# JiLiBIT/LIO-SLAM

Measured on AMD Instinct MI355X. Metric: scan-to-map registrations/sec, 64x1800 scan vs 200-keyframe map; pose RMSE, higher is better.
Workload: dtype f32

## Files before the change

### include/liogpu.h

```cpp
#ifndef LIOGPU_H
#define LIOGPU_H

#include <stddef.h>
#include <stdint.h>

#ifdef __cplusplus
extern "C" {
#endif

#define LIO_VERSION 102
#define LIO_MAX_ITERS 32

enum {
    LIO_OK               = 0,
    LIO_TOO_FEW_POINTS   = 1,
    LIO_TOO_FEW_CORR     = 2,
    LIO_ERR_ARG          = -1,
    LIO_ERR_HIP          = -2,
    LIO_ERR_CAPACITY     = -3,
    LIO_ERR_NO_MAP       = -4,
    LIO_ERR_NO_DEVICE    = -5
};

typedef struct lio_s2m_config {
// ... 99 lines not shown
void  lio_host_free(void *p);
int   lio_host_register(void *p, size_t bytes);
int   lio_host_unregister(void *p);
void *lio_device_alloc(int32_t device_id, size_t bytes);
void  lio_device_free(int32_t device_id, void *p);
int   lio_device_upload(int32_t device_id, void *dst, const void *src, size_t bytes);

int  lio_s2m_set_degeneracy(lio_s2m_handle *h, int32_t scan, const float matP[36], int32_t is_degenerate);

int  lio_s2m_get_correspondences(lio_s2m_handle *h, int32_t scan, uint8_t *flag,
                                 float *coeff4, int32_t *nn_idx5);

int  lio_s2m_set_corner_map(lio_s2m_handle *h, const void *pts, size_t n, size_t stride_bytes);
int  lio_s2m_batch_upload_corners(lio_s2m_handle *h, int32_t n_scans, const void *const *scans,
                                  const size_t *n_pts, size_t stride_bytes);
int  lio_s2m_register_cs(lio_s2m_handle *h, const void *corner_scan, size_t n_corner,
                         const void *surf_scan, size_t n_surf, size_t stride_bytes,
                         float pose[6], lio_s2m_result *res);
int  lio_s2m_get_corner_correspondences(lio_s2m_handle *h, int32_t scan, uint8_t *flag,
                                        float *coeff4, int32_t *nn_idx5);

int  lio_s2m_get_profile(lio_s2m_handle *h, lio_s2m_profile *out);
int  lio_s2m_debug_persist_spin(lio_s2m_handle *h, int32_t spin_max, int32_t withhold_wg);
int  lio_s2m_debug_stamps(lio_s2m_handle *h, long long *out, size_t cap_entries);

int  lio_s2m_set_stream(lio_s2m_handle *h, void *hip_stream);
int  lio_s2m_set_global_grid(lio_s2m_handle *h, const float origin[3], const int32_t dims[3]);
int  lio_s2m_set_shard(lio_s2m_handle *h, int32_t axis, int32_t lo, int32_t hi);
int  lio_s2m_set_shard_plan(lio_s2m_handle *h, int32_t axis, int32_t n_ranks, int32_t rank, const int32_t *bounds,
                            int32_t halo_cells);
int  lio_s2m_set_scan_shard(lio_s2m_handle *h, int32_t rank, int32_t world);
int  lio_s2m_batch_begin(lio_s2m_handle *h);
int  lio_s2m_batch_iter_partial(lio_s2m_handle *h, double *d_sums );
int  lio_s2m_batch_iter_apply(lio_s2m_handle *h, const double *d_sums);
int  lio_s2m_batch_n_active(lio_s2m_handle *h, int32_t *n_active);
int  lio_s2m_batch_poll_active(lio_s2m_handle *h, int32_t iteration, int32_t *n_active);

void lio_transform_update(float pose[6], int32_t imu_available, int32_t imu_type,
                          float imu_roll_init, float imu_pitch_init, float imu_rpy_weight,
                          float rotation_tollerance, float z_tollerance);

typedef struct lio_deskew_config {
    int32_t N_SCAN;
    int32_t downsampleRate;
    int32_t point_filter_num;
    float   lidarMinFront, lidarMinBack, lidarMinLeft, lidarMinRight;
// ... 113 lines not shown
```

### lio-slam_amd/api.py

```python
import ctypes as C
import os
import subprocess

import numpy as np

_HERE = os.path.dirname(os.path.abspath(__file__))
LIO_MAX_ITERS = 32
STATUS_NAMES = {0: "OK", 1: "TOO_FEW_POINTS", 2: "TOO_FEW_CORR", -1: "ERR_ARG", -2: "ERR_HIP",
                -3: "ERR_CAPACITY", -4: "ERR_NO_MAP", -5: "ERR_NO_DEVICE"}


class LioError(RuntimeError):
    pass


class S2MConfig(C.Structure):
    _fields_ = [
        ("k", C.c_int32), ("max_sq_dist", C.c_float),
        ("plane_tol", C.c_double), ("weight", C.c_double), ("min_s", C.c_double),
        ("min_corr", C.c_int32), ("max_iters", C.c_int32), ("eig_thresh", C.c_float),
        ("conv_deg", C.c_double), ("conv_cm", C.c_double),
        ("min_scan_pts", C.c_int32), ("jacobian_mode", C.c_int32), ("force_all_iters", C.c_int32),
        ("device_id", C.c_int32), ("cell_size", C.c_float), ("max_batch", C.c_int32),
        ("max_scan_pts", C.c_int32), ("record_corr_iter", C.c_int32), ("kernel_variant", C.c_int32),
# ... 72 lines not shown
    if verbose:
        print(out.stdout)
    return lib_path()


_LIB = None

EXPORTS = [
    "lio_version", "lio_s2m_default_config", "lio_last_error", "lio_s2m_create", "lio_s2m_destroy",
    "lio_s2m_set_map", "lio_s2m_register", "lio_s2m_batch_upload", "lio_s2m_batch_set_poses",
    "lio_s2m_batch_run", "lio_s2m_batch_sync", "lio_s2m_batch_results", "lio_s2m_set_degeneracy",
    "lio_s2m_get_correspondences", "lio_s2m_get_profile", "lio_s2m_set_stream",
    "lio_s2m_set_global_grid", "lio_s2m_set_shard", "lio_s2m_batch_begin",
    "lio_s2m_batch_iter_partial", "lio_s2m_batch_iter_apply", "lio_s2m_batch_n_active",
    "lio_transform_update", "lio_deskew_default_config", "lio_imu_deskew_info", "lio_deskew",
    "lio_curvature", "lio_s2m_debug_stamps", "lio_s2m_batch_poll_active", "lio_voxel_grid", "lio_assemble_map", "lio_kf_store_create", "lio_kf_store_destroy", "lio_kf_store_add",
    "lio_kf_store_count", "lio_kf_store_points", "lio_assemble_map_resident", "lio_s2m_set_scan_shard",
    "lio_s2m_set_corner_map", "lio_s2m_batch_upload_corners", "lio_s2m_register_cs",
    "lio_s2m_get_corner_correspondences", "lio_feature_default_config", "lio_extract_features",
    "lio_range_image_default_config", "lio_range_image",
    "lio_s2m_share_map", "lio_s2m_batch_upload_async", "lio_host_alloc", "lio_host_free", "lio_host_register",
    "lio_host_unregister", "lio_s2m_set_shard_plan", "lio_s2m_register_pc2", "lio_deskew_pc2", "lio_kf_store_add_device", "lio_kf_store_add_from_handle",
    "lio_s2m_register_raw", "lio_s2m_debug_persist_spin", "lio_device_alloc", "lio_device_free", "lio_device_upload",
    "lio_nearby_default_config", "lio_kf_store_set_poses", "lio_assemble_map_nearby",
]


def load_library():
    global _LIB
    if _LIB is not None:
        return _LIB
    p = lib_path()
    if not os.path.exists(p):
        raise LioError(f"{p} is missing: run __graft_entry__.build() (hipcc --offload-arch=gfx950). "
                       "There is no CPU fallback.")
    L = C.CDLL(p)
    vp, i32, f32, f64, sz = C.c_void_p, C.c_int32, C.c_float, C.c_double, C.c_size_t
    L.lio_version.restype = C.c_int
    L.lio_last_error.restype = C.c_char_p
    L.lio_s2m_default_config.argtypes = [C.POINTER(S2MConfig)]
    L.lio_s2m_default_config.restype = None
    L.lio_s2m_create.argtypes = [C.POINTER(S2MConfig), C.POINTER(vp)]
    L.lio_s2m_destroy.argtypes = [vp]
    L.lio_s2m_destroy.restype = None
    L.lio_s2m_set_map.argtypes = [vp, vp, sz, sz]
    L.lio_s2m_register.argtypes = [vp, vp, sz, sz, C.POINTER(f32), C.POINTER(S2MResult)]
    L.lio_s2m_register_pc2.argtypes = [vp, vp, sz, C.POINTER(PC2Layout), C.POINTER(f32), C.POINTER(S2MResult)]
# ... 421 lines not shown
                            dp(T), dp(RX), dp(RY), dp(RZ), cur, out.ctypes.data, 32, C.byref(n_out)), "lio_deskew_pc2")
    o = out[:n_out.value]
    return np.concatenate([o[:, :3], o[:, 4:5]], axis=1).copy()


def deskew_default_config(**kw):
    c = DeskewConfig()
    load_library().lio_deskew_default_config(C.byref(c))
    for k, v in kw.items():
        setattr(c, k, v)
    return c


def curvature(rng, device_id=0):
    r = np.ascontiguousarray(rng, np.float32)
    curv = np.zeros(len(r), np.float32)
    picked = np.full(len(r), -1, np.int32)
    label = np.full(len(r), -1, np.int32)
    _check(load_library().lio_curvature(device_id, r.ctypes.data, len(r), curv.ctypes.data,
                                        picked.ctypes.data, label.ctypes.data), "lio_curvature")
    return curv, picked, label


def range_image(records, t_cur, imu, device_id=0, **cfg_overrides):
    L = load_library()
    cfg = RangeImageConfig()
    L.lio_range_image_default_config(C.byref(cfg))
    cfg.device_id = device_id
    for k, v in cfg_overrides.items():
        if not hasattr(cfg, k):
            raise AttributeError(k)
        setattr(cfg, k, v)
    cur, T, RX, RY, RZ = imu
    rec = np.ascontiguousarray(records)
    cells = int(cfg.N_SCAN) * int(cfg.Horizon_SCAN)
    out = _scratch("ri_cloud", (max(cells, 1), 8))
    col = _scratch("ri_col", (max(cells, 1),), np.int32)
    rng = _scratch("ri_range", (max(cells, 1),))
    start = np.zeros(cfg.N_SCAN, np.int32)
    end = np.zeros(cfg.N_SCAN, np.int32)
    n_out = C.c_size_t()
    dpp = lambda a: a.ctypes.data_as(C.POINTER(C.c_double))
    _check(L.lio_range_image(C.byref(cfg), rec.ctypes.data, len(rec), rec.dtype.itemsize, t_cur, dpp(T), dpp(RX), dpp(RY), dpp(RZ),
                             cur, out.ctypes.data, 32, C.byref(n_out), start.ctypes.data, end.ctypes.data, col.ctypes.data,
                             rng.ctypes.data), "lio_range_image")
    n = n_out.value
# ... 156 lines not shown
```

### lio-slam_amd/csrc/lio_device_math.h

```cpp
#pragma once
#include <hip/hip_runtime.h>
#include <float.h>
#include <stdint.h>

#define LIO_DEV __device__ __forceinline__

LIO_DEV void lio_plane_qr5x3(float a[5][3], float x[3])
{
    float hc[3], direct[3], upd[3];
    int trans[3];
#pragma unroll
    for (int k = 0; k < 3; ++k) {
        float s = 0.0f;
#pragma unroll
        for (int i = 0; i < 5; ++i) s += a[i][k] * a[i][k];
        direct[k] = sqrtf(s);
        upd[k] = direct[k];
    }
    float maxn = upd[0];
    if (upd[1] > maxn) maxn = upd[1];
    if (upd[2] > maxn) maxn = upd[2];
    const float th = maxn * FLT_EPSILON;
    const float threshold_helper = (th * th) / 5.0f;
    const float downdate_thr = sqrtf(FLT_EPSILON);
    int nz = 3;

#pragma unroll
    for (int k = 0; k < 3; ++k) {
// ... 10 lines not shown
            const bool sw = (big == j);
#pragma unroll
            for (int i = 0; i < 5; ++i) {
                const float u = a[i][k], v = a[i][j];
                a[i][k] = sw ? v : u;
                a[i][j] = sw ? u : v;
            }
            const float u0 = upd[k], u1 = upd[j], d0 = direct[k], d1 = direct[j];
            upd[k] = sw ? u1 : u0;       upd[j] = sw ? u0 : u1;
            direct[k] = sw ? d1 : d0;    direct[j] = sw ? d0 : d1;
        }
        float tail_sq = 0.0f;
#pragma unroll
        for (int i = k + 1; i < 5; ++i) tail_sq += a[i][k] * a[i][k];
        const float c0 = a[k][k];
        float beta, tau;
        if (tail_sq <= FLT_MIN) {
            tau = 0.0f; beta = c0;
#pragma unroll
            for (int i = k + 1; i < 5; ++i) a[i][k] = 0.0f;
        } else {
            beta = sqrtf(c0 * c0 + tail_sq);
            if (c0 >= 0.0f) beta = -beta;
            const float den = c0 - beta;
#pragma unroll
            for (int i = k + 1; i < 5; ++i) a[i][k] = a[i][k] / den;
            tau = (beta - c0) / beta;
        }
        hc[k] = tau;
        a[k][k] = beta;
        if (tau != 0.0f) {
#pragma unroll
            for (int j = k + 1; j < 3; ++j) {
                float tmp = 0.0f;
#pragma unroll
                for (int i = k + 1; i < 5; ++i) tmp += a[i][k] * a[i][j];
                tmp += a[k][j];
                a[k][j] -= tau * tmp;
#pragma unroll
                for (int i = k + 1; i < 5; ++i) a[i][j] -= (tau * a[i][k]) * tmp;
            }
        }
#pragma unroll
        for (int j = k + 1; j < 3; ++j) {
            if (upd[j] != 0.0f) {
                float temp = fabsf(a[k][j]) / upd[j];
                temp = (1.0f + temp) * (1.0f - temp);
                temp = temp < 0.0f ? 0.0f : temp;
                const float ratio = upd[j] / direct[j];
// ... 37 lines not shown
                tmp += c[k];
                c[k] -= tau * tmp;
#pragma unroll
                for (int i = k + 1; i < 5; ++i) c[i] -= (tau * a[i][k]) * tmp;
            }
        }
    }
#pragma unroll
    for (int i = 2; i >= 0; --i) {
        if (i < nz) {
            if (c[i] != 0.0f) {
                c[i] /= a[i][i];
#pragma unroll
                for (int r = 0; r < i; ++r) c[r] -= c[i] * a[r][i];
            }
        }
    }
    const float v0 = (0 < nz) ? c[0] : 0.0f;
    const float v1 = (1 < nz) ? c[1] : 0.0f;
    const float v2 = (2 < nz) ? c[2] : 0.0f;
#pragma unroll
    for (int j = 0; j < 3; ++j)
        x[j] = (p0 == j) ? v0 : (p1 == j) ? v1 : (p2 == j) ? v2 : 0.0f;
}

LIO_DEV void lio_jacobian_row(const float tr[6], float px, float py, float pz,
                              float cx, float cy, float cz, float cw, int jac_exact,
                              float row[6], float &rhs)
{
    const float srx = tr[0], crx = tr[1], sry = tr[2], cry = tr[3], srz = tr[4], crz = tr[5];
    const float arx = (-srx * cry * px - (srx * sry * srz + crx * crz) * py + (crx * srz - srx * sry * crz) * pz) * cx
                    + (crx * cry * px - (srx * crz - crx * sry * srz) * py + (crx * sry * crz + srx * srz) * pz) * cy;
    const float mid = jac_exact ? (srx * cry * srz * py) : (srx * sry * srz * py);
    const float ary = (-crx * sry * px + crx * cry * srz * py + crx * cry * crz * pz) * cx
                    + (-srx * sry * px + mid + srx * cry * crz * pz) * cy
                    + (-cry * px - sry * srz * py - sry * crz * pz) * cz;
    const float arz = ((crx * sry * crz + srx * srz) * py + (srx * crz - crx * sry * srz) * pz) * cx
                    + ((-crx * srz + srx * sry * crz) * py + (-srx * sry * srz - crx * crz) * pz) * cy
                    + (cry * crz * py - cry * srz * pz) * cz;
    row[0] = arz; row[1] = ary; row[2] = arx;
    row[3] = cx;  row[4] = cy;  row[5] = cz;
    rhs = -cw;
}

__device__ static float lio_cv_hypot(float a, float b)
{
// ... 369 lines not shown
```

### lio-slam_amd/csrc/lio_kernels.h

```cpp
#pragma once
#include <hip/hip_runtime.h>
#include "lio_types.h"

struct LioIterParams {
    LioGrid grid;
    LioShard shard;
    LioConsts c;
    const float4* map_sorted;
    const float4* map_xyz4;
    const int* cell_start;
    const float4* nbr_pts;
    const int* nbr_start;
    const float* sx;
    const float* sy;
    const float* sz;
    const int* perm;
    LioScanState* state;
    const LioBlockDesc* blocks;
    double* partials;
    unsigned* arrive;
    int max_blk;
    int xcd_remap;
    int* n_active;
    double* sums_out;
// ... 17 lines not shown
                           int* n_active, hipStream_t s);
void lio_launch_iterate(const LioIterParams& P, int n_blocks, int ppt, bool stage, hipStream_t s, bool corner = false);
void lio_launch_persist(const LioIterParams& P, int n_blocks, unsigned* gen, unsigned epoch, const unsigned char* stage, size_t stride,
                        int n_scans, unsigned* spec, double* spec_sums, const float* poses0, unsigned spin_max, int withhold_wg, hipStream_t s);
void lio_launch_pack_summary(const LioScanState* st, int n_scans, float* out, hipStream_t s);
void lio_launch_apply(LioScanState* st, int n_scans, const double* sums, size_t slot_stride, int n_slots, const LioConsts& c,
                      int* n_active, hipStream_t s);
void lio_launch_shard_cull(const LioIterParams& P, int n_ranks, int rank, int halo, const int* bounds, const float* block_box,
                           int n_blocks, unsigned char* skip, hipStream_t s);
void lio_launch_block_boxes(const LioBlockDesc* blocks, int n_blocks, const LioScanState* st, const float* sx, const float* sy,
                            const float* sz, float* box, hipStream_t s);
void lio_launch_scan_sort_lds(const void* stage, size_t stride, const LioScanState* st, int n_scans, int max_pts, float tile0,
                              int shard_axis, int* perm, float* x, float* y, float* z, hipStream_t s);
void lio_launch_scan_bbox(const void* stage, size_t stride, const LioBlockDesc* prep_blocks, int n_prep_blocks,
                          const LioScanState* st, unsigned* bbox, hipStream_t s);
void lio_launch_scan_tile_sort(const void* stage, size_t stride, int total_pts,
                               const LioBlockDesc* prep_blocks, int n_prep_blocks,
                               const LioScanState* st, const LioScanTiles* tiles, int n_keys,
                               int* key_of, int* key_count, int* key_start, int* tile_sums,
                               int* tmp_idx, int* perm, int* big_list, int* big_cnt,
                               float* x, float* y, float* z, hipStream_t s);
void lio_launch_exclusive_scan(const int* in, int n, int* tile_sums, int* out, hipStream_t s);
void lio_launch_xyzi4_to_soa(const float4* src, int n, float* x, float* y, float* z, float4* xyz4, hipStream_t s);
```

### lio-slam_amd/csrc/lio_kernels.hip

```cpp
#include <hip/hip_runtime.h>
#include "lio_types.h"
#include "lio_device_math.h"
#include "lio_kernels.h"

#include "lio_s2m_device.h"
#include "lio_scan2.h"

LIO_DEV unsigned lio_f2ord(float f)
{
    unsigned u = __float_as_uint(f);
    return (u & 0x80000000u) ? ~u : (u | 0x80000000u);
}

__global__ void k_aos_to_soa(const unsigned char* __restrict__ src, size_t stride, int n,
                             float* __restrict__ x, float* __restrict__ y, float* __restrict__ z,
                             float4* __restrict__ xyz4 )
{
    int i = blockIdx.x * blockDim.x + threadIdx.x;
    if (i >= n) return;
    const float* p = reinterpret_cast<const float*>(src + (size_t)i * stride);
    const float a = p[0], b = p[1], c = p[2];
    x[i] = a; y[i] = b; z[i] = c;
    if (xyz4) xyz4[i] = make_float4(a, b, c, 0.0f);
}
// ... 704 lines not shown
__global__ __launch_bounds__(LIO_BLOCK, (PPT == 1 && !STAGE && !CORNER) ? LIO_MIN_WAVES : 4) void k_s2m_iterate(LioIterParams P)
{
    __shared__ __attribute__((aligned(16))) double s_rows[LIO_BLOCK][8];
    __shared__ double s_part[8][28];
    __shared__ double s_sum[28];
    __shared__ LioSolveWs s_ws;
    __shared__ __attribute__((aligned(16))) float4 s_pts[STAGE ? LIO_LDS_PTS : 1];
    __shared__ int s_cell[STAGE ? LIO_LDS_CELLS : 1];
    __shared__ int s_row_beg[STAGE ? LIO_LDS_ROWS : 1];
    __shared__ int s_row_off[STAGE ? LIO_LDS_ROWS + 1 : 1];
    __shared__ int s_box[8];
    __shared__ int s_scan4[4];

    int wg = blockIdx.x;
    if (P.xcd_remap) {
        const int n8 = gridDim.x >> 3;
        if (wg < n8 * 8) wg = (wg & 7) * n8 + (wg >> 3);
    }
    const int wg_mode = P.blk_skip != nullptr ? (int)P.blk_skip[wg] : 0;
    if (wg_mode == 1) return;
    const LioBlockDesc bd = P.blocks[wg];
    LioScanState* st = &P.state[bd.scan];
    if (st->done) return;
    long long* stamp = P.stamps ? P.stamps + ((size_t)wg * (LIO_BLOCK / 64) + (threadIdx.x >> 6)) * 8 : nullptr;
#define LIO_STAMP(k) do { if (stamp && (threadIdx.x & 63) == 0) stamp[k] = (long long)__builtin_readcyclecounter(); } while (0)
    LIO_STAMP(0);

    float T[12], tr[6];
#pragma unroll
    for (int k = 0; k < 12; ++k) T[k] = st->T[k];
#pragma unroll
    for (int k = 0; k < 6; ++k) tr[k] = st->trig[k];
    const int n_pts = CORNER ? st->c_n_pts : st->n_pts;
    const int base = CORNER ? st->c_offset : st->offset;
    const bool record = (P.rec_flag != nullptr) && (st->iter == P.c.record_iter);
    const bool use_cache = (P.d5_cache != nullptr) && !STAGE && st->iter > 0;
    float Tp[12];
#pragma unroll
    for (int k = 0; k < 12; ++k) Tp[k] = use_cache ? st->Tp[k] : 0.0f;
    const LioGrid g = P.grid;
    const int lane = threadIdx.x & 63, wave = threadIdx.x >> 6;

    float px[PPT], py[PPT], pz[PPT], qx[PPT], qy[PPT], qz[PPT];
    int cx[PPT], cy[PPT], cz[PPT];
    bool act[PPT], inr[PPT];
    int bmn[3] = { 0x7fffffff, 0x7fffffff, 0x7fffffff }, bmx[3] = { -0x7fffffff, -0x7fffffff, -0x7fffffff };
#pragma unroll
    for (int pp = 0; pp < PPT; ++pp) {
        const int li = bd.first + pp * LIO_BLOCK + (int)threadIdx.x;
        inr[pp] = li < n_pts;
        const int gi = base + (inr[pp] ? li : 0);
        px[pp] = P.sx[gi]; py[pp] = P.sy[gi]; pz[pp] = P.sz[gi];
        qx[pp] = T[0] * px[pp] + T[1] * py[pp] + T[2]  * pz[pp] + T[3];
        qy[pp] = T[4] * px[pp] + T[5] * py[pp] + T[6]  * pz[pp] + T[7];
        qz[pp] = T[8] * px[pp] + T[9] * py[pp] + T[10] * pz[pp] + T[11];
        bool a = inr[pp];
        if (P.shard.axis >= 0 && wg_mode != 2) {
            const float qa = P.shard.axis == 0 ? qx[pp] : (P.shard.axis == 1 ? qy[pp] : qz[pp]);
            int gc = lio_cell_coord(qa, P.shard.gorigin, P.shard.inv_cell, P.shard.gdim);
            gc = min(max(gc, 0), P.shard.gdim - 1);
            a = a && gc >= P.shard.lo && gc < P.shard.hi;
        }
// ... 80 lines not shown
                }
                for (int i = threadIdx.x; i < total; i += LIO_BLOCK) {
                    int lo = 0, hi = n_rows - 1;
                    while (lo < hi) {
                        const int mid = (lo + hi + 1) >> 1;
                        if (s_row_off[mid] <= i) lo = mid; else hi = mid - 1;
                    }
                    s_pts[i] = P.map_sorted[s_row_beg[lo] + (i - s_row_off[lo])];
                }
                staged = true;
            }
            __syncthreads();
        }
    }

    const int red_g = threadIdx.x >> 5, red_s = threadIdx.x & 31;
    const int red_a = c_pair_a[red_s], red_b = c_pair_b[red_s];
    double red_acc = 0.0;
    LIO_STAMP(1);

#pragma unroll 1
    for (int pp = 0; pp < PPT; ++pp) {
        float bound2 = P.c.max_sq_dist;
        float Rx = sqrtf(P.c.max_sq_dist) * 1.0001f + 1e-6f;
        bool bounded = false;
        const int ci = base + bd.first + pp * LIO_BLOCK + (int)threadIdx.x;
        if (use_cache && act[pp]) {
            const float d5 = P.d5_cache[ci];
            if (d5 >= 0.0f) {
                const float ox = Tp[0] * px[pp] + Tp[1] * py[pp] + Tp[2]  * pz[pp] + Tp[3];
                const float oy = Tp[4] * px[pp] + Tp[5] * py[pp] + Tp[6]  * pz[pp] + Tp[7];
                const float oz = Tp[8] * px[pp] + Tp[9] * py[pp] + Tp[10] * pz[pp] + Tp[11];
                const float mv = sqrtf(lio_sqdist(qx[pp], qy[pp], qz[pp], ox, oy, oz));
                const float R = (sqrtf(d5) + mv) * 1.0001f + 1e-6f;
                const float r2 = R * R * 1.0001f;
                if (r2 < bound2) { bound2 = r2; Rx = R; bounded = true; }
            }
        }
        const double sentinel = lio_make_key(bound2, -1);
        LioTop5 top = { sentinel, sentinel, sentinel, sentinel, sentinel };
        if (act[pp]) {
            if (STAGE && staged)
                lio_knn_lds(s_pts, s_cell, rxn1, ryn, rx0, ry0, rz0, ry1, rz1, g.nx, g.k,
                            qx[pp], qy[pp], qz[pp], cx[pp], cy[pp], cz[pp], top);
            else
                lio_knn_global(P, g, qx[pp], qy[pp], qz[pp], cy[pp], cz[pp], Rx, bound2, bounded, top);
        }
// ... 29 lines not shown
        __syncthreads();
        if (red_s < 28) {
#pragma unroll 8
            for (int p = red_g; p < LIO_BLOCK; p += 8)
                red_acc = __builtin_fma(s_rows[p][red_a], s_rows[p][red_b], red_acc);
        }
    }
    LIO_STAMP(4);
    if (red_s < 28) s_part[red_g][red_s] = red_acc;
    __syncthreads();
    LIO_STAMP(5);
    if (wave != 0) return;

    double* part = P.partials + ((size_t)bd.scan * P.max_blk + bd.blk) * LIO_SUMS;
    if (lane < 28) {
        double v = s_part[0][lane];
#pragma unroll
        for (int w = 1; w < 8; ++w) v += s_part[w][lane];
        __hip_atomic_store(part + lane, v, __ATOMIC_RELAXED, __HIP_MEMORY_SCOPE_AGENT);
    }
    lio_arrive_and_finish(P, bd, st, lane, s_sum, &s_ws, stamp);
    LIO_STAMP(7);
#undef LIO_STAMP
}

__global__ void k_s2m_pack_summary(const LioScanState* __restrict__ st, int n_scans, float* __restrict__ out)
{
    const int s = blockIdx.x * blockDim.x + threadIdx.x;
    if (s >= n_scans) return;
    float* o = out + (size_t)s * 10;
    for (int k = 0; k < 6; ++k) o[k] = st[s].pose[k];
    o[6] = __int_as_float(st[s].iter); o[7] = __int_as_float(st[s].status | (st[s].done ? 0 : 0x100));
    o[8] = __int_as_float(st[s].converged); o[9] = __int_as_float(st[s].is_degenerate);
}

__global__ void k_s2m_apply(LioScanState* __restrict__ st, int n_scans, const double* __restrict__ sums, size_t slot_stride, int n_slots,
                            LioConsts c, int* __restrict__ n_active)
{
    const int s = blockIdx.x;
    if (s >= n_scans) return;
    if (st[s].done) return;
    __shared__ LioSolveWs s_ws;
    __shared__ double s_tot[LIO_SUMS];
    const int lane = (int)threadIdx.x;
    if (lane < LIO_SUMS) {
        const double* p = sums + (size_t)s * LIO_SUMS + lane;
// ... 205 lines not shown
```

### lio-slam_amd/csrc/lio_persist.hip

```cpp
#include <hip/hip_runtime.h>
#ifndef LIO_PREFETCH
#define LIO_PREFETCH 2
#endif
#include "lio_kernels.h"
#include "lio_device_math.h"
#include "lio_s2m_device.h"

namespace {

__global__ __launch_bounds__(LIO_BLOCK, 2) void k_s2m_persist(LioIterParams P, unsigned* __restrict__ gen, unsigned epoch, const unsigned char* __restrict__ stage, unsigned stride,
                   int n_main, unsigned* __restrict__ spec, double* __restrict__ spec_sums, const float* __restrict__ poses0,
                   unsigned spin_max, int withhold_wg)
{
    __shared__ __attribute__((aligned(16))) double s_rows[LIO_BLOCK][8];
    __shared__ double s_part[8][28];
    __shared__ double s_sum[28];
    __shared__ LioSolveWs s_ws;
    __shared__ int s_ctl;

    const int wg = blockIdx.x;
    if (wg >= n_main) {
        const int scan = wg - n_main;
        if (threadIdx.x >= 64) return;
        const int hl = threadIdx.x;
// ... 72 lines not shown
        float T[12], tr[6], Tp[12];
#pragma unroll
        for (int k = 0; k < 12; ++k) T[k] = st->T[k];
#pragma unroll
        for (int k = 0; k < 6; ++k) tr[k] = st->trig[k];
        const int st_iter = st->iter;
        const bool record = (P.rec_flag != nullptr) && (st_iter == P.c.record_iter);
        const bool use_cache = (P.d5_cache != nullptr) && st_iter > 0;
#pragma unroll
        for (int k = 0; k < 12; ++k) Tp[k] = use_cache ? st->Tp[k] : 0.0f;

        const float qx = T[0] * px + T[1] * py + T[2]  * pz + T[3];
        const float qy = T[4] * px + T[5] * py + T[6]  * pz + T[7];
        const float qz = T[8] * px + T[9] * py + T[10] * pz + T[11];
        const int cx = lio_cell_coord(qx, g.ox, g.inv_cell, g.nx);
        const int cy = lio_cell_coord(qy, g.oy, g.inv_cell, g.ny);
        const int cz = lio_cell_coord(qz, g.oz, g.inv_cell, g.nz);
        bool act = inr;
        act = act && (fabsf(qx) <= 3.0e38f) && (fabsf(qy) <= 3.0e38f) && (fabsf(qz) <= 3.0e38f);
        act = act && cx >= -g.k && cx < g.nx + g.k && cy >= -g.k && cy < g.ny + g.k && cz >= -g.k && cz < g.nz + g.k;

        LIO_TICK(0);
        float bound2 = P.c.max_sq_dist;
        float Rx = sqrtf(P.c.max_sq_dist) * 1.0001f + 1e-6f;
        bool bounded = false;
        if (use_cache && act) {
            const float d5 = P.d5_cache[ci];
            if (d5 >= 0.0f) {
                const float ox = Tp[0] * px + Tp[1] * py + Tp[2]  * pz + Tp[3];
                const float oy = Tp[4] * px + Tp[5] * py + Tp[6]  * pz + Tp[7];
                const float oz = Tp[8] * px + Tp[9] * py + Tp[10] * pz + Tp[11];
                const float mv = sqrtf(lio_sqdist(qx, qy, qz, ox, oy, oz));
                const float R = (sqrtf(d5) + mv) * 1.0001f + 1e-6f;
                const float r2 = R * R * 1.0001f;
                if (r2 < bound2) { bound2 = r2; Rx = R; bounded = true; }
            }
        }
        const double sentinel = lio_make_key(bound2, -1);
        LioTop5 top = { sentinel, sentinel, sentinel, sentinel, sentinel };
        if (act) lio_knn_global(P, g, qx, qy, qz, cy, cz, Rx, bound2, bounded, top);
        const bool ok = act && (lio_key_d2(top.k4) < P.c.max_sq_dist);
        const int nn[5] = { lio_key_idx(top.k0), lio_key_idx(top.k1), lio_key_idx(top.k2), lio_key_idx(top.k3), lio_key_idx(top.k4) };
        if (P.d5_cache && inr) P.d5_cache[ci] = ok ? lio_key_d2(top.k4) : -1.0f;
        LIO_TICK(1);

        float cxx = 0.0f, cyy = 0.0f, czz = 0.0f, cww = 0.0f;
        bool accept = false;
// ... 150 lines not shown
```

### lio-slam_amd/csrc/lio_s2m_device.h

```cpp
#pragma once
#include <hip/hip_runtime.h>
#include "lio_types.h"
#include "lio_device_math.h"
#include "lio_kernels.h"

#define LIO_MAX_COORD 1.0e15f
#ifndef LIO_PREFETCH
#define LIO_PREFETCH 1
#endif
#ifndef LIO_ARRIVE_ACQREL
#define LIO_ARRIVE_ACQREL 0
#endif
#define LIO_IDX_MASK 0x1fffffff

LIO_DEV int lio_cell_coord(float v, float origin, float inv_cell, int n)
{
    float c = floorf((v - origin) * inv_cell);
    c = fminf(fmaxf(c, -4.0f), (float)(n + 3));
    return (int)c;
}

LIO_DEV double lio_dmin(double a, double b) { double r; asm("v_min_f64 %0, %1, %2" : "=v"(r) : "v"(a), "v"(b)); return r; }
LIO_DEV double lio_dmax(double a, double b) { double r; asm("v_max_f64 %0, %1, %2" : "=v"(r) : "v"(a), "v"(b)); return r; }

// ... 154 lines not shown
    return 0;
}

typedef float lio_f2 __attribute__((ext_vector_type(2)));

LIO_DEV void lio_knn_pair(const float4& a, const float4& b, lio_f2 qx, lio_f2 qy, lio_f2 qz, double& k0, double& k1)
{
    const lio_f2 X = { a.x, a.y }, Y = { a.z, a.w }, Z = { b.x, b.y };
    const lio_f2 dx = X - qx, dy = Y - qy, dz = Z - qz;
    const lio_f2 d2 = (dx * dx + dy * dy) + dz * dz;
    k0 = lio_make_key(d2.x, __float_as_int(b.z));
    k1 = lio_make_key(d2.y, __float_as_int(b.w));
}

LIO_DEV void lio_knn_group(const float4& c0, const float4& c1, const float4& c2, const float4& c3,
                           lio_f2 qx, lio_f2 qy, lio_f2 qz, LioTop5& top)
{
    double k0, k1, k2, k3;
    lio_knn_pair(c0, c1, qx, qy, qz, k0, k1);
    lio_knn_pair(c2, c3, qx, qy, qz, k2, k3);
    lio_top5_insert4(top, k0, k1, k2, k3);
}

LIO_DEV void lio_knn_range(const LioIterParams& P, const LioGrid& g, float qx, float qy, float qz,
                           int cy, int cz, float Rx, unsigned& beg, unsigned& end)
{
    const int xlo = lio_cell_coord(qx - Rx, g.ox, g.inv_cell_x, g.nxf), xhi = lio_cell_coord(qx + Rx, g.ox, g.inv_cell_x, g.nxf);
    const int x0 = max(xlo, 0), x1 = min(xhi, g.nxf - 1);
    beg = end = 0;
    if (x0 > x1) return;
    int row = (min(max(cz, 0), g.nz - 1) * g.ny + min(max(cy, 0), g.ny - 1)) * g.nxf;
#pragma unroll
    for (int l = 0; l < LIO_TB_MAX; ++l) {
        if (Rx <= g.tb_reach[l]) {
            const int by = min(max(lio_cell_coord(qy, g.tb_oy[l], g.tb_inv_cell[l], g.tb_ny[l]), 0), g.tb_ny[l] - 1);
            const int bz = min(max(lio_cell_coord(qz, g.tb_oz[l], g.tb_inv_cell[l], g.tb_nz[l]), 0), g.tb_nz[l] - 1);
            row = g.tb_row0[l] + (bz * g.tb_ny[l] + by) * g.nxf;
        }
    }
#if LIO_PREFETCH == 3
    beg = (unsigned)P.nbr_start[row + x0] & ~7u;
#else
    beg = (unsigned)P.nbr_start[row + x0] & ~3u;
#endif
    end = (unsigned)P.nbr_start[row + x1 + 1];
}

LIO_DEV void lio_knn_run(const LioIterParams& P, unsigned beg, unsigned end, float qx, float qy, float qz, LioTop5& top)
{
    if (beg >= end) return;
    const lio_f2 QX = { qx, qx }, QY = { qy, qy }, QZ = { qz, qz };
    const float4* p = P.nbr_pts + beg;
#if LIO_PREFETCH == 2
    float4 c0 = p[0], c1 = p[1], c2 = p[2], c3 = p[3];
    float4 n0 = p[4], n1 = p[5], n2 = p[6], n3 = p[7];
    for (unsigned j = beg;;) {
        float4 f0 = n0, f1 = n1, f2 = n2, f3 = n3;
        if (j + 8 < end) { f0 = p[8]; f1 = p[9]; f2 = p[10]; f3 = p[11]; }
        lio_knn_group(c0, c1, c2, c3, QX, QY, QZ, top);
        j += 4;
        if (j >= end) break;
        p += 4;
// ... 12 lines not shown
        const float4 b0 = p[4], b1 = p[5], b2 = p[6], b3 = p[7];
        lio_knn_group(a0, a1, a2, a3, QX, QY, QZ, top);
        p += 8;
        a0 = p[0]; a1 = p[1]; a2 = p[2]; a3 = p[3];
        lio_knn_group(b0, b1, b2, b3, QX, QY, QZ, top);
        j += 8;
    } while (j < end);
#else
    float4 c0 = p[0], c1 = p[1], c2 = p[2], c3 = p[3];
    for (unsigned j = beg + 4; j < end; j += 4) {
        p += 4;
        const float4 n0 = p[0], n1 = p[1], n2 = p[2], n3 = p[3];
        lio_knn_group(c0, c1, c2, c3, QX, QY, QZ, top);
        c0 = n0; c1 = n1; c2 = n2; c3 = n3;
    }
    lio_knn_group(c0, c1, c2, c3, QX, QY, QZ, top);
#endif
}

LIO_DEV void lio_knn_global(const LioIterParams& P, const LioGrid& g, float qx, float qy, float qz,
                            int cy, int cz, float Rx, float bound2, bool bounded, LioTop5& top)
{
    int lvl = bounded ? -1 : g.tb_try;
    for (;;) {
        float rx = Rx, b2 = bound2;
        if (lvl >= 0) {
            rx = lvl == 2 ? g.tb_reach[2] : (lvl == 1 ? g.tb_reach[1] : g.tb_reach[0]);
            b2 = lvl == 2 ? g.tb_try_b2[2] : (lvl == 1 ? g.tb_try_b2[1] : g.tb_try_b2[0]);
        }
        const double sentinel = lio_make_key(b2, -1);
        top.k0 = top.k1 = top.k2 = top.k3 = top.k4 = sentinel;
        unsigned beg, end;
        lio_knn_range(P, g, qx, qy, qz, cy, cz, rx, beg, end);
        lio_knn_run(P, beg, end, qx, qy, qz, top);
        if (lvl < 0 || lio_key_idx(top.k4) != -1) break;
        --lvl;
    }
}

template <bool CORNER>
LIO_DEV bool lio_assoc_point(const LioIterParams& P, const int nn[5], float qx, float qy, float qz,
                             float px, float py, float pz, float& cxx, float& cyy, float& czz, float& cww)
{
    bool accept = false;
    float a[5][3], m[5][3];
#pragma unroll
    for (int j = 0; j < 5; ++j) {
        const float4 mp = P.map_xyz4[nn[j]];
        m[j][0] = a[j][0] = mp.x;
        m[j][1] = a[j][1] = mp.y;
        m[j][2] = a[j][2] = mp.z;
    }
    if (CORNER) {
        accept = lio_corner_assoc(m, qx, qy, qz, P.c.weight, P.c.min_s, cxx, cyy, czz, cww);
    } else {
        float X0[3];
        lio_plane_qr5x3(a, X0);
        float pa = X0[0], pb = X0[1], pc = X0[2], pd = 1;
        const float ps = sqrtf(pa * pa + pb * pb + pc * pc);
        pa /= ps; pb /= ps; pc /= ps; pd /= ps;
        bool planeValid = true;
#pragma unroll
        for (int j = 0; j < 5; ++j) {
            const float v = fabsf(pa * m[j][0] + pb * m[j][1] + pc * m[j][2] + pd);
            if ((double)v > P.c.plane_tol) planeValid = false;
        }
        if (planeValid) {
            const float pd2 = pa * qx + pb * qy + pc * qz + pd;
            const float r2 = px * px + py * py + pz * pz;
            const float s = (float)(1 - P.c.weight * (double)fabsf(pd2) / (double)sqrtf(sqrtf(r2)));
            cxx = s * pa; cyy = s * pb; czz = s * pc; cww = s * pd2;
            accept = (double)s > P.c.min_s;
        }
    }
    return accept;
}

static __constant__ int c_pair_a[32] = { 0,0,0,0,0,0, 1,1,1,1,1, 2,2,2,2, 3,3,3, 4,4, 5,  0,1,2,3,4,5, 7, 0,0,0,0 };
static __constant__ int c_pair_b[32] = { 0,1,2,3,4,5, 1,2,3,4,5, 2,3,4,5, 3,4,5, 4,5, 5,  6,6,6,6,6,6, 7, 0,0,0,0 };

LIO_DEV void lio_arrive_and_finish(const LioIterParams& P, const LioBlockDesc& bd, LioScanState* st, int lane,
                                   double* s_sum, LioSolveWs* s_ws, long long* stamp)
{
#if !LIO_ARRIVE_ACQREL
    asm volatile("s_waitcnt vmcnt(0)" ::: "memory");
#endif
    int last = 0;
    if (lane == 0) {
#if LIO_ARRIVE_ACQREL
// ... 31 lines not shown
```

### lio-slam_amd/csrc/lio_types.h

```cpp
#pragma once
#include <stdint.h>

#define LIO_SUMS 32
#define LIO_SUM_NC 27
#define LIO_BLOCK 256
#define LIO_ROW_ALIGN 8

#define LIO_TB_MAX 3
struct LioGrid {
    float ox, oy, oz;
    float inv_cell;
    int32_t nx, ny, nz;
    int32_t n_cells;
    int32_t k;
    int32_t xs;
    int32_t nxf;
    float inv_cell_x;
    int32_t tb_row0[LIO_TB_MAX], tb_ny[LIO_TB_MAX], tb_nz[LIO_TB_MAX];
    float tb_oy[LIO_TB_MAX], tb_oz[LIO_TB_MAX], tb_inv_cell[LIO_TB_MAX], tb_reach[LIO_TB_MAX];
    int32_t tb_try;
    float tb_try_b2[LIO_TB_MAX];
};

struct LioShard {
    float gorigin;
    float inv_cell;
    int32_t axis;
    int32_t gdim;
    int32_t lo, hi;
};

struct LioConsts {
    double plane_tol, weight, min_s, conv_deg, conv_cm;
    float  max_sq_dist, eig_thresh;
    int32_t min_corr, max_iters, jac_exact, force_all, record_iter, min_scan_pts;
};

struct LioScanState {
    float pose[6];
    float T[12];
    float Tp[12];
    float trig[6];
    int32_t n_pts;
    int32_t offset;
    int32_t c_n_pts;
    int32_t c_offset;
    int32_t iter;
    int32_t done;
    int32_t converged;
    int32_t is_degenerate;
    int32_t n_corr_last;
    int32_t status;
    float matP[36];
    float AtA[36];
    float AtB[6];
    int32_t n_corr_iter[32];
    float pose_iter[32][6];
// ... 17 lines not shown
```

### lio-slam_amd/csrc/liogpu_api.hip

```cpp
#include <hip/hip_runtime.h>
#include <math.h>
#include <stdio.h>
#include <string.h>
#include <algorithm>
#include <chrono>
#include <exception>
#include <memory>
#include <mutex>
#include <vector>

#include "lio_handle.h"
#include "lio_multi.h"


static thread_local char g_last_error[512];

int lio_fail(int code, const char* what, hipError_t e)
{
    if (e != hipSuccess) snprintf(g_last_error, sizeof(g_last_error), "%s: %s", what, hipGetErrorString(e));
    else snprintf(g_last_error, sizeof(g_last_error), "%s", what);
    return code;
}

int lio_fail_exception(void)
// ... 38 lines not shown
    c->lookahead = -1;
    c->use_lds = 0;
    c->cell_div = 2;
    c->xcd_remap = 1;
    c->tile_size = 0.0f;
    c->use_graph = 0;
    c->sort_batch = 1;
    c->graph_iters = 4;
    c->sort_scan = 1;
    c->nn_cache = 1;
    c->pipeline = 0;
    c->n_devices = 1;
    for (int i = 0; i < 8; ++i) c->device_ids[i] = i;
    c->x_sub = 0;
    c->tight_rows = 0;
}

static void lio_fill_consts(lio_s2m_handle* h)
{
    const lio_s2m_config& g = h->cfg;
    h->c.plane_tol = g.plane_tol; h->c.weight = g.weight; h->c.min_s = g.min_s;
    h->c.conv_deg = g.conv_deg; h->c.conv_cm = g.conv_cm;
    h->c.max_sq_dist = g.max_sq_dist; h->c.eig_thresh = g.eig_thresh;
    h->c.min_corr = g.min_corr; h->c.max_iters = g.max_iters;
    h->c.jac_exact = g.jacobian_mode ? 1 : 0; h->c.force_all = g.force_all_iters ? 1 : 0;
    h->c.record_iter = g.record_corr_iter; h->c.min_scan_pts = g.min_scan_pts;
}

static int lio_s2m_init_resources(lio_s2m_handle* h)
{
    HIPCHK(hipStreamCreateWithFlags(&h->stream, hipStreamNonBlocking));
    for (int i = 0; i < LIO_MAX_ITERS; ++i) {
        HIPCHK(hipEventCreate(&h->ev_beg[i]));
        HIPCHK(hipEventCreate(&h->ev_end[i]));
        HIPCHK(hipEventCreateWithFlags(&h->ev_chk[i], hipEventDisableTiming));
    }
    HIPCHK(h->h_active.grow(LIO_MAX_ITERS, LIO_MAX_ITERS));
    HIPCHK(hipEventCreate(&h->ev_map[0]));
    HIPCHK(hipEventCreate(&h->ev_map[1]));
    HIPCHK(hipEventCreate(&h->ev_mapl[0]));
    HIPCHK(hipEventCreate(&h->ev_mapl[1]));
    HIPCHK(h->d_bbox.grow(6, 1.0, 0));
    HIPCHK(h->d_active.grow(1, 1.0, 0));
    hipDeviceProp_t prop;
    if (hipGetDeviceProperties(&prop, h->cfg.device_id) == hipSuccess) h->n_cu = prop.multiProcessorCount;
    (void)hipGetLastError();
// ... 409 lines not shown
} LIO_CATCH

static bool lio_persist_eligible(const lio_s2m_handle* h)
{
    int limit = 0;
    if (h->cfg.pipeline == 4) limit = h->n_cu;
    else if (h->cfg.pipeline == 0 && !h->cfg.use_graph && h->cfg.profile != 2) limit = h->n_cu / 2;
    return limit > 0 && !h->no_persist && !h->cfg.use_lds && h->ppt == 1 && h->shard.axis < 0 &&
           h->block_world == 1 && h->n_blocks > 0 && h->n_blocks + h->n_scans <= limit;
}

static unsigned lio_persist_spin_max(const lio_s2m_handle* h)
{
    if (h->persist_spin_max) return h->persist_spin_max;
    static const unsigned env = [] { const char* e = getenv("LIO_PERSIST_SPIN_MAX"); const long v = e ? atol(e) : 0; return v > 0 ? (unsigned)v : 4096u; }();
    return env;
}

extern "C" int lio_s2m_debug_persist_spin(lio_s2m_handle* h, int32_t spin_max, int32_t withhold_wg)
try {
    if (!h) return lio_fail(LIO_ERR_ARG, "null handle");
    h->persist_spin_max = spin_max > 0 ? (unsigned)spin_max : 0u;
    h->persist_withhold = withhold_wg;
    return LIO_OK;
} LIO_CATCH

static int lio_ensure_soa(lio_s2m_handle* h)
{
    if (h->soa_valid || !h->total_pts) return LIO_OK;
    lio_launch_aos_to_soa(h->last_stage + h->last_xyz_off, h->last_stride, (int)h->total_pts, h->d_sx, h->d_sy, h->d_sz, nullptr, h->stream);
    h->soa_valid = true;
    HIPCHK(hipGetLastError());
    return LIO_OK;
}

extern "C" int lio_s2m_batch_upload(lio_s2m_handle* h, int32_t n_scans, const void* const* scans,
                                    const size_t* n_pts, size_t stride)
try {
    if (!h || !scans || !n_pts) return lio_fail(LIO_ERR_ARG, "null argument");
    if (n_scans < 1) return lio_fail(LIO_ERR_ARG, "n_scans must be >= 1");
    if (stride < 12 || (stride & 3)) return lio_fail(LIO_ERR_ARG, "stride_bytes must be >= 12 and a multiple of 4");
    if (h->multi) return lio_multi_upload(h, n_scans, scans, n_pts, stride);
    HIPCHK(hipSetDevice(h->cfg.device_id));
    (void)hipGetLastError();
    size_t total = 0, max_n = 0;
    for (int s = 0; s < n_scans; ++s) {
// ... 1017 lines not shown
```

Measured before the change: 423,000.

## Share reciprocal divisions in plane fit, hoist gate reach and coarse-row lookup

Replaces the repeated per-element divisions in the Householder QR and in plane normalisation with one refined reciprocal plus Newton-corrected multiplies, guarded by range checks so the result matches true division. Precomputes the sqrt-based gate reach on the host and computes the coarse-table row indices once per query rather than on every retry level of the KNN range search. Also hoists the scan-state loads ahead of the stamp and adds a debug plane-fit kernel and API for checking the results. The extra range checks and the per-query row array add some instructions and register pressure.

```diff
diff --git a/include/liogpu.h b/include/liogpu.h
--- a/include/liogpu.h
+++ b/include/liogpu.h
@@ -145,6 +145,8 @@
 
 int  lio_s2m_get_profile(lio_s2m_handle *h, lio_s2m_profile *out);
 int  lio_s2m_debug_persist_spin(lio_s2m_handle *h, int32_t spin_max, int32_t withhold_wg);
+
+int  lio_debug_plane_fit(int32_t device_id, const float *sets, size_t n, double plane_tol, uint32_t *out);
 int  lio_s2m_debug_stamps(lio_s2m_handle *h, long long *out, size_t cap_entries);
 
 int  lio_s2m_set_stream(lio_s2m_handle *h, void *hip_stream);
diff --git a/lio-slam_amd/api.py b/lio-slam_amd/api.py
--- a/lio-slam_amd/api.py
+++ b/lio-slam_amd/api.py
@@ -118,7 +118,7 @@
     "lio_s2m_share_map", "lio_s2m_batch_upload_async", "lio_host_alloc", "lio_host_free", "lio_host_register",
     "lio_host_unregister", "lio_s2m_set_shard_plan", "lio_s2m_register_pc2", "lio_deskew_pc2", "lio_kf_store_add_device", "lio_kf_store_add_from_handle",
     "lio_s2m_register_raw", "lio_s2m_debug_persist_spin", "lio_device_alloc", "lio_device_free", "lio_device_upload",
-    "lio_nearby_default_config", "lio_kf_store_set_poses", "lio_assemble_map_nearby",
+    "lio_nearby_default_config", "lio_kf_store_set_poses", "lio_assemble_map_nearby", "lio_debug_plane_fit",
 ]
 
 
@@ -586,6 +586,15 @@
     return curv, picked, label
 
 
+def debug_plane_fit(sets, plane_tol=0.2, device_id=0):
+    a = np.ascontiguousarray(sets, np.float32).reshape(-1, 15)
+    out = np.zeros((len(a), 8), np.uint32)
+    fn = load_library().lio_debug_plane_fit
+    fn.argtypes = [C.c_int32, C.c_void_p, C.c_size_t, C.c_double, C.c_void_p]
+    _check(fn(device_id, a.ctypes.data, len(a), float(plane_tol), out.ctypes.data), "lio_debug_plane_fit")
+    return out
+
+
 def range_image(records, t_cur, imu, device_id=0, **cfg_overrides):
     L = load_library()
     cfg = RangeImageConfig()
diff --git a/lio-slam_amd/csrc/lio_device_math.h b/lio-slam_amd/csrc/lio_device_math.h
--- a/lio-slam_amd/csrc/lio_device_math.h
+++ b/lio-slam_amd/csrc/lio_device_math.h
@@ -4,6 +4,35 @@
 #include <stdint.h>
 
 #define LIO_DEV __device__ __forceinline__
+
+#ifndef LIO_SHARED_DIV
+#define LIO_SHARED_DIV 1
+#endif
+struct LioDivisor { float d, r; bool mid; };
+
+LIO_DEV bool lio_div_mid(float lo, float hi) { return lo >= 0x1p-40f && hi < 0x1p40f; }
+
+LIO_DEV LioDivisor lio_divisor(float d)
+{
+    LioDivisor v;
+    const float r0 = __builtin_amdgcn_rcpf(d);
+    const float e = __builtin_fmaf(-d, r0, 1.0f);
+    v.d = d; v.r = __builtin_fmaf(e, r0, r0);
+    v.mid = lio_div_mid(fabsf(d), fabsf(d));
+    return v;
+}
+
+LIO_DEV float lio_div_fast(float n, const LioDivisor& v)
+{
+    float q = n * v.r;
+    float e = __builtin_fmaf(-v.d, q, n);
+    q = __builtin_fmaf(e, v.r, q);
+    e = __builtin_fmaf(-v.d, q, n);
+    return __builtin_fmaf(e, v.r, q);
+}
+
+LIO_DEV float lio_min3_abs(float a, float b, float c) { return fminf(fminf(fabsf(a), fabsf(b)), fabsf(c)); }
+LIO_DEV float lio_max3_abs(float a, float b, float c) { return fmaxf(fmaxf(fabsf(a), fabsf(b)), fabsf(c)); }
 
 LIO_DEV void lio_plane_qr5x3(float a[5][3], float x[3])
 {
@@ -60,9 +89,17 @@
         } else {
             beta = sqrtf(c0 * c0 + tail_sq);
             if (c0 >= 0.0f) beta = -beta;
-            const float den = c0 - beta;
-#pragma unroll
-            for (int i = k + 1; i < 5; ++i) a[i][k] = a[i][k] / den;
+            const LioDivisor den = lio_divisor(c0 - beta);
+            float lo = fabsf(a[k + 1][k]), hi = lo;
+#pragma unroll
+            for (int i = k + 2; i < 5; ++i) { lo = fminf(lo, fabsf(a[i][k])); hi = fmaxf(hi, fabsf(a[i][k])); }
+            if (LIO_SHARED_DIV && den.mid && lio_div_mid(lo, hi)) {
+#pragma unroll
+                for (int i = k + 1; i < 5; ++i) a[i][k] = lio_div_fast(a[i][k], den);
+            } else {
+#pragma unroll
+                for (int i = k + 1; i < 5; ++i) a[i][k] = a[i][k] / den.d;
+            }
             tau = (beta - c0) / beta;
         }
         hc[k] = tau;
@@ -146,6 +183,29 @@
 #pragma unroll
     for (int j = 0; j < 3; ++j)
         x[j] = (p0 == j) ? v0 : (p1 == j) ? v1 : (p2 == j) ? v2 : 0.0f;
+}
+
+LIO_DEV bool lio_plane_fit5(const float m[5][3], double plane_tol, float X0[3], float& pa, float& pb, float& pc, float& pd)
+{
+    float a[5][3];
+#pragma unroll
+    for (int j = 0; j < 5; ++j) { a[j][0] = m[j][0]; a[j][1] = m[j][1]; a[j][2] = m[j][2]; }
+    lio_plane_qr5x3(a, X0);
+    pa = X0[0]; pb = X0[1]; pc = X0[2]; pd = 1;
+    const float ps = sqrtf(pa * pa + pb * pb + pc * pc);
+    const LioDivisor dv = lio_divisor(ps);
+    if (LIO_SHARED_DIV && dv.mid && lio_div_mid(lio_min3_abs(pa, pb, pc), lio_max3_abs(pa, pb, pc))) {
+        pa = lio_div_fast(pa, dv); pb = lio_div_fast(pb, dv); pc = lio_div_fast(pc, dv); pd = lio_div_fast(pd, dv);
+    } else {
+        pa /= ps; pb /= ps; pc /= ps; pd /= ps;
+    }
+    bool planeValid = true;
+#pragma unroll
+    for (int j = 0; j < 5; ++j) {
+        const float v = fabsf(pa * m[j][0] + pb * m[j][1] + pc * m[j][2] + pd);
+        if ((double)v > plane_tol) planeValid = false;
+    }
+    return planeValid;
 }
 
 LIO_DEV void lio_jacobian_row(const float tr[6], float px, float py, float pz,
diff --git a/lio-slam_amd/csrc/lio_kernels.h b/lio-slam_amd/csrc/lio_kernels.h
--- a/lio-slam_amd/csrc/lio_kernels.h
+++ b/lio-slam_amd/csrc/lio_kernels.h
@@ -63,3 +63,4 @@
                                float* x, float* y, float* z, hipStream_t s);
 void lio_launch_exclusive_scan(const int* in, int n, int* tile_sums, int* out, hipStream_t s);
 void lio_launch_xyzi4_to_soa(const float4* src, int n, float* x, float* y, float* z, float4* xyz4, hipStream_t s);
+void lio_launch_debug_plane_fit(const float* sets, long long n, double plane_tol, unsigned* out, hipStream_t s);
diff --git a/lio-slam_amd/csrc/lio_kernels.hip b/lio-slam_amd/csrc/lio_kernels.hip
--- a/lio-slam_amd/csrc/lio_kernels.hip
+++ b/lio-slam_amd/csrc/lio_kernels.hip
@@ -750,22 +750,23 @@
     const LioBlockDesc bd = P.blocks[wg];
     LioScanState* st = &P.state[bd.scan];
     if (st->done) return;
+    float T[12], tr[6];
+#pragma unroll
+    for (int k = 0; k < 12; ++k) T[k] = st->T[k];
+#pragma unroll
+    for (int k = 0; k < 6; ++k) tr[k] = st->trig[k];
+    float Tp[12];
+#pragma unroll
+    for (int k = 0; k < 12; ++k) Tp[k] = st->Tp[k];
+    const int n_pts = CORNER ? st->c_n_pts : st->n_pts;
+    const int base = CORNER ? st->c_offset : st->offset;
+    const int st_iter = st->iter;
     long long* stamp = P.stamps ? P.stamps + ((size_t)wg * (LIO_BLOCK / 64) + (threadIdx.x >> 6)) * 8 : nullptr;
 #define LIO_STAMP(k) do { if (stamp && (threadIdx.x & 63) == 0) stamp[k] = (long long)__builtin_readcyclecounter(); } while (0)
     LIO_STAMP(0);
 
-    float T[12], tr[6];
-#pragma unroll
-    for (int k = 0; k < 12; ++k) T[k] = st->T[k];
-#pragma unroll
-    for (int k = 0; k < 6; ++k) tr[k] = st->trig[k];
-    const int n_pts = CORNER ? st->c_n_pts : st->n_pts;
-    const int base = CORNER ? st->c_offset : st->offset;
-    const bool record = (P.rec_flag != nullptr) && (st->iter == P.c.record_iter);
-    const bool use_cache = (P.d5_cache != nullptr) && !STAGE && st->iter > 0;
-    float Tp[12];
-#pragma unroll
-    for (int k = 0; k < 12; ++k) Tp[k] = use_cache ? st->Tp[k] : 0.0f;
+    const bool record = (P.rec_flag != nullptr) && (st_iter == P.c.record_iter);
+    const bool use_cache = (P.d5_cache != nullptr) && !STAGE && st_iter > 0;
     const LioGrid g = P.grid;
     const int lane = threadIdx.x & 63, wave = threadIdx.x >> 6;
 
@@ -892,7 +893,7 @@
 #pragma unroll 1
     for (int pp = 0; pp < PPT; ++pp) {
         float bound2 = P.c.max_sq_dist;
-        float Rx = sqrtf(P.c.max_sq_dist) * 1.0001f + 1e-6f;
+        float Rx = P.c.gate_reach;
         bool bounded = false;
         const int ci = base + bd.first + pp * LIO_BLOCK + (int)threadIdx.x;
         if (use_cache && act[pp]) {
@@ -968,6 +969,29 @@
     lio_arrive_and_finish(P, bd, st, lane, s_sum, &s_ws, stamp);
     LIO_STAMP(7);
 #undef LIO_STAMP
+}
+
+__global__ __launch_bounds__(256) void k_debug_plane_fit(const float* __restrict__ sets, long long n, double plane_tol,
+                                                         unsigned* __restrict__ out)
+{
+    const long long i = (long long)blockIdx.x * 256 + threadIdx.x;
+    if (i >= n) return;
+    float m[5][3];
+#pragma unroll
+    for (int j = 0; j < 5; ++j)
+#pragma unroll
+        for (int c = 0; c < 3; ++c) m[j][c] = sets[i * 15 + j * 3 + c];
+    float X0[3], pa, pb, pc, pd;
+    const bool valid = lio_plane_fit5(m, plane_tol, X0, pa, pb, pc, pd);
+    uint4* o = reinterpret_cast<uint4*>(out + i * 8);
+    o[0] = make_uint4(__float_as_uint(X0[0]), __float_as_uint(X0[1]), __float_as_uint(X0[2]), __float_as_uint(pa));
+    o[1] = make_uint4(__float_as_uint(pb), __float_as_uint(pc), __float_as_uint(pd), valid ? 1u : 0u);
+}
+
+void lio_launch_debug_plane_fit(const float* sets, long long n, double plane_tol, unsigned* out, hipStream_t s)
+{
+    if (n <= 0) return;
+    hipLaunchKernelGGL(k_debug_plane_fit, dim3((unsigned)((n + 255) / 256)), dim3(256), 0, s, sets, n, plane_tol, out);
 }
 
 __global__ void k_s2m_pack_summary(const LioScanState* __restrict__ st, int n_scans, float* __restrict__ out)
diff --git a/lio-slam_amd/csrc/lio_persist.hip b/lio-slam_amd/csrc/lio_persist.hip
--- a/lio-slam_amd/csrc/lio_persist.hip
+++ b/lio-slam_amd/csrc/lio_persist.hip
@@ -118,7 +118,7 @@
 
         LIO_TICK(0);
         float bound2 = P.c.max_sq_dist;
-        float Rx = sqrtf(P.c.max_sq_dist) * 1.0001f + 1e-6f;
+        float Rx = P.c.gate_reach;
         bool bounded = false;
         if (use_cache && act) {
             const float d5 = P.d5_cache[ci];
diff --git a/lio-slam_amd/csrc/lio_s2m_device.h b/lio-slam_amd/csrc/lio_s2m_device.h
--- a/lio-slam_amd/csrc/lio_s2m_device.h
+++ b/lio-slam_amd/csrc/lio_s2m_device.h
@@ -200,8 +200,23 @@
     lio_top5_insert4(top, k0, k1, k2, k3);
 }
 
-LIO_DEV void lio_knn_range(const LioIterParams& P, const LioGrid& g, float qx, float qy, float qz,
-                           int cy, int cz, float Rx, unsigned& beg, unsigned& end)
+LIO_DEV void lio_tb_rows(const LioGrid& g, float qy, float qz, int (&tb_row)[LIO_TB_MAX])
+{
+#pragma unroll
+    for (int l = 0; l < LIO_TB_MAX; ++l) {
+        tb_row[l] = 0;
+        if (g.tb_reach[l] > 0.0f) {
+            const int by = min(max(lio_cell_coord(qy, g.tb_oy[l], g.tb_inv_cell[l], g.tb_ny[l]), 0), g.tb_ny[l] - 1);
+            const int bz = min(max(lio_cell_coord(qz, g.tb_oz[l], g.tb_inv_cell[l], g.tb_nz[l]), 0), g.tb_nz[l] - 1);
+            int row = g.tb_row0[l] + (bz * g.tb_ny[l] + by) * g.nxf;
+            asm volatile("" : "+v"(row));
+            tb_row[l] = row;
+        }
+    }
+}
+
+LIO_DEV void lio_knn_range(const LioIterParams& P, const LioGrid& g, float qx, int cy, int cz, const int (&tb_row)[LIO_TB_MAX],
+                           float Rx, unsigned& beg, unsigned& end)
 {
     const int xlo = lio_cell_coord(qx - Rx, g.ox, g.inv_cell_x, g.nxf), xhi = lio_cell_coord(qx + Rx, g.ox, g.inv_cell_x, g.nxf);
     const int x0 = max(xlo, 0), x1 = min(xhi, g.nxf - 1);
@@ -209,13 +224,8 @@
     if (x0 > x1) return;
     int row = (min(max(cz, 0), g.nz - 1) * g.ny + min(max(cy, 0), g.ny - 1)) * g.nxf;
 #pragma unroll
-    for (int l = 0; l < LIO_TB_MAX; ++l) {
-        if (Rx <= g.tb_reach[l]) {
-            const int by = min(max(lio_cell_coord(qy, g.tb_oy[l], g.tb_inv_cell[l], g.tb_ny[l]), 0), g.tb_ny[l] - 1);
-            const int bz = min(max(lio_cell_coord(qz, g.tb_oz[l], g.tb_inv_cell[l], g.tb_nz[l]), 0), g.tb_nz[l] - 1);
-            row = g.tb_row0[l] + (bz * g.tb_ny[l] + by) * g.nxf;
-        }
-    }
+    for (int l = 0; l < LIO_TB_MAX; ++l)
+        if (Rx <= g.tb_reach[l]) row = tb_row[l];
 #if LIO_PREFETCH == 3
     beg = (unsigned)P.nbr_start[row + x0] & ~7u;
 #else
@@ -274,6 +284,8 @@
                             int cy, int cz, float Rx, float bound2, bool bounded, LioTop5& top)
 {
     int lvl = bounded ? -1 : g.tb_try;
+    int tb_row[LIO_TB_MAX];
+    lio_tb_rows(g, qy, qz, tb_row);
     for (;;) {
         float rx = Rx, b2 = bound2;
         if (lvl >= 0) {
@@ -283,7 +295,7 @@
         const double sentinel = lio_make_key(b2, -1);
         top.k0 = top.k1 = top.k2 = top.k3 = top.k4 = sentinel;
         unsigned beg, end;
-        lio_knn_range(P, g, qx, qy, qz, cy, cz, rx, beg, end);
+        lio_knn_range(P, g, qx, cy, cz, tb_row, rx, beg, end);
         lio_knn_run(P, beg, end, qx, qy, qz, top);
         if (lvl < 0 || lio_key_idx(top.k4) != -1) break;
         --lvl;
@@ -295,28 +307,17 @@
                              float px, float py, float pz, float& cxx, float& cyy, float& czz, float& cww)
 {
     bool accept = false;
-    float a[5][3], m[5][3];
+    float m[5][3];
 #pragma unroll
     for (int j = 0; j < 5; ++j) {
         const float4 mp = P.map_xyz4[nn[j]];
-        m[j][0] = a[j][0] = mp.x;
-        m[j][1] = a[j][1] = mp.y;
-        m[j][2] = a[j][2] = mp.z;
+        m[j][0] = mp.x; m[j][1] = mp.y; m[j][2] = mp.z;
     }
     if (CORNER) {
         accept = lio_corner_assoc(m, qx, qy, qz, P.c.weight, P.c.min_s, cxx, cyy, czz, cww);
     } else {
-        float X0[3];
-        lio_plane_qr5x3(a, X0);
-        float pa = X0[0], pb = X0[1], pc = X0[2], pd = 1;
-        const float ps = sqrtf(pa * pa + pb * pb + pc * pc);
-        pa /= ps; pb /= ps; pc /= ps; pd /= ps;
-        bool planeValid = true;
-#pragma unroll
-        for (int j = 0; j < 5; ++j) {
-            const float v = fabsf(pa * m[j][0] + pb * m[j][1] + pc * m[j][2] + pd);
-            if ((double)v > P.c.plane_tol) planeValid = false;
-        }
+        float X0[3], pa, pb, pc, pd;
+        const bool planeValid = lio_plane_fit5(m, P.c.plane_tol, X0, pa, pb, pc, pd);
         if (planeValid) {
             const float pd2 = pa * qx + pb * qy + pc * qz + pd;
             const float r2 = px * px + py * py + pz * pz;
diff --git a/lio-slam_amd/csrc/lio_types.h b/lio-slam_amd/csrc/lio_types.h
--- a/lio-slam_amd/csrc/lio_types.h
+++ b/lio-slam_amd/csrc/lio_types.h
@@ -33,6 +33,7 @@
 struct LioConsts {
     double plane_tol, weight, min_s, conv_deg, conv_cm;
     float  max_sq_dist, eig_thresh;
+    float  gate_reach;
     int32_t min_corr, max_iters, jac_exact, force_all, record_iter, min_scan_pts;
 };
 
diff --git a/lio-slam_amd/csrc/liogpu_api.hip b/lio-slam_amd/csrc/liogpu_api.hip
--- a/lio-slam_amd/csrc/liogpu_api.hip
+++ b/lio-slam_amd/csrc/liogpu_api.hip
@@ -84,6 +84,12 @@
     h->c.plane_tol = g.plane_tol; h->c.weight = g.weight; h->c.min_s = g.min_s;
     h->c.conv_deg = g.conv_deg; h->c.conv_cm = g.conv_cm;
     h->c.max_sq_dist = g.max_sq_dist; h->c.eig_thresh = g.eig_thresh;
+    {
+        volatile float r = sqrtf(g.max_sq_dist);
+        r = r * 1.0001f;
+        r = r + 1e-6f;
+        h->c.gate_reach = r;
+    }
     h->c.min_corr = g.min_corr; h->c.max_iters = g.max_iters;
     h->c.jac_exact = g.jacobian_mode ? 1 : 0; h->c.force_all = g.force_all_iters ? 1 : 0;
     h->c.record_iter = g.record_corr_iter; h->c.min_scan_pts = g.min_scan_pts;
@@ -539,6 +545,23 @@
     if (!h) return lio_fail(LIO_ERR_ARG, "null handle");
     h->persist_spin_max = spin_max > 0 ? (unsigned)spin_max : 0u;
     h->persist_withhold = withhold_wg;
+    return LIO_OK;
+} LIO_CATCH
+
+extern "C" int lio_debug_plane_fit(int32_t device_id, const float* sets, size_t n, double plane_tol, uint32_t* out)
+try {
+    if ((!sets || !out) && n) return lio_fail(LIO_ERR_ARG, "null pointer");
+    if (n > ((size_t)1 << 27)) return lio_fail(LIO_ERR_CAPACITY, "at most 2^27 sets per call");
+    if (!n) return LIO_OK;
+    HIPCHK(hipSetDevice(device_id));
+    LioDevBuf<float> d_sets;
+    LioDevBuf<unsigned> d_out;
+    HIPCHK(d_sets.grow(n * 15, 1.0, 0));
+    HIPCHK(d_out.grow(n * 8, 1.0, 0));
+    HIPCHK(hipMemcpy(d_sets, sets, n * 15 * sizeof(float), hipMemcpyHostToDevice));
+    lio_launch_debug_plane_fit(d_sets, (long long)n, plane_tol, d_out, nullptr);
+    HIPCHK(hipGetLastError());
+    HIPCHK(hipMemcpy(out, d_out, n * 8 * sizeof(unsigned), hipMemcpyDeviceToHost));
     return LIO_OK;
 } LIO_CATCH
 
```

After: 438,900, median of 6. +3.8%, better.
